# Chen001117/mappo

Hardware: AMD Instinct MI355X
Metric: agent-steps/sec (collect+GAE+PPO), MPE simple_spread 3-agent (higher is better)
Workload: dtype f32; 1 GPU; BASELINE configs[1]: MPE simple_spread shape, 3 agents, obs 18 / share_obs 54 / Discrete(5), n_rollout_threads=1024 in total (strong scaling: 1024 on rank 0 of 1), episode_length=25, MLP policy (mappo), ppo_epoch=10, num_mini_batch=1, lr 7e-4, env=synthetic; n_rollout_threads_global=1024, n_rollout_threads_rank0=1024, episode_length=25, num_agents=3, ppo_epoch=10, num_mini_batch=1, parallelism=dp1, rccl_ranks=0, exact_minibatch_order=False, hip_graph=True

## Files before the change

### include/mappo_hip.h

```cpp
#ifndef MAPPO_HIP_H
#define MAPPO_HIP_H

#include <stdint.h>

#ifdef __cplusplus
extern "C" {
#endif

typedef void *mappo_stream_t;

#define MAPPO_OK 0
#define MAPPO_EINVAL (-1)
#define MAPPO_ELAUNCH (-2)
#define MAPPO_ENOTIMPL (-3)

#define MAPPO_HIDDEN 64
#define MAPPO_MAX_IN_DIM 512
#define MAPPO_MAX_ACTIONS 32
#define MAPPO_MAX_LAYER_N 2

const char *mappo_last_error(void);
int mappo_abi_version(void);

typedef struct {
// ... 126 lines not shown
                       mappo_stream_t stream);
int mappo_critic_update(const float *params, const mappo_net_desc *desc , const float *share_obs,
                        const int32_t *rows, int64_t B, const float *v_old, const float *returns,
                        const float *active, const float *vn_state ,
                        const double *mb_moments , const mappo_ppo_cfg *cfg , float *slabs,
                        int64_t slab_stride, int64_t slab_col0, double *partials, float *wide_ws ,
                        int32_t n_blocks, mappo_stream_t stream);
int32_t mappo_dual_update_slabs(const mappo_net_desc *actor_desc , const mappo_net_desc *critic_desc , int64_t B);
int mappo_actor_critic_update(const float *actor_params, const mappo_net_desc *actor_desc , const float *obs,
                              const float *critic_params, const mappo_net_desc *critic_desc , const float *share_obs,
                              const int32_t *rows, int64_t B, const float *avail, const float *actions, const float *old_logp,
                              const float *adv, const float *active, const float *v_old, const float *returns,
                              const float *vn_state, const double *mb_moments, const mappo_ppo_cfg *cfg , float *slabs,
                              int64_t slab_stride, int64_t actor_col0, int64_t critic_col0, double *actor_partials,
                              double *critic_partials, mappo_stream_t stream);
int mappo_update_stats(const double *actor_partials, int32_t n_actor ,
                       const double *critic_partials, int32_t n_critic, const double *mb_moments,
                       const mappo_ppo_cfg *cfg , double *stats ,
                       double *acc ,
                       mappo_stream_t stream);

int mappo_mlp_features(const float *params, const mappo_net_desc *desc , const float *x, const int32_t *rows,
                       int64_t B, float *featT , mappo_stream_t stream);
int mappo_gru_forward(const float *params, const mappo_net_desc *desc , const float *featT, const float *h0,
                      const int32_t *h0_rows , const float *masks, const int32_t *rows ,
                      int32_t L, int32_t Nc, float *h_last ,
                      int32_t head_mode, float *out, const float *avail , int32_t deterministic,
                      uint64_t seed, uint64_t counter, const uint64_t *counter_dev, float *actions, float *logp,
                      mappo_stream_t stream);
int mappo_gru_step_dual(const float *actor_params, const mappo_net_desc *actor_desc , const float *actor_featT ,
// ... 94 lines not shown
```

### mappo_amd/_lib.py

```python
import ctypes as C
import os

import torch

_HERE = os.path.dirname(os.path.abspath(__file__))
LIB_PATH = os.environ.get("MAPPO_HIP_LIB") or os.path.join(_HERE, "libmappo_hip.so")

HIDDEN = 64
MAX_ACTIONS = 32
MAX_LAYER_N = 2


class NetDesc(C.Structure):
    _fields_ = [("in_dim", C.c_int32), ("hidden", C.c_int32), ("out_dim", C.c_int32), ("layer_N", C.c_int32),
                ("use_relu", C.c_int32), ("use_feature_norm", C.c_int32), ("recurrent", C.c_int32)]


class PpoCfg(C.Structure):
    _fields_ = [("clip_param", C.c_float), ("entropy_coef", C.c_float), ("value_loss_coef", C.c_float),
                ("huber_delta", C.c_float), ("use_huber_loss", C.c_int32), ("use_clipped_value_loss", C.c_int32),
                ("use_policy_active_masks", C.c_int32), ("use_value_active_masks", C.c_int32),
                ("use_valuenorm", C.c_int32), ("accumulate_partials", C.c_int32)]


# ... 32 lines not shown
                                        _I64, _I64, _P, _I64, _I64, _I64, _I32, _U64, _U64, _P, _P, _P, _P, _P, _P, _P, _P, _P, _I32, _P]),
    "mappo_mlp_backward_slabs": (_I32, [_I64]),
    "mappo_mlp_backward": (C.c_int, [_P, C.POINTER(NetDesc), _P, _P, _I64, _P, _P, _I64, _I64, _P, _P]),
    "mappo_wide_workspace_floats": (_I64, [_I64]),
    "mappo_wide_l1_slabs": (_I32, [_I64]),
    "mappo_wide_layout": (_I32, [C.POINTER(NetDesc), _I32]),
    "mappo_wide_l1_backward": (C.c_int, [_P, C.POINTER(NetDesc), _P, _P, _I64, _P, _P, _I64, _I64, _I32, _P]),
    "mappo_update_partials_bytes": (_I64, []),
    "mappo_actor_update": (C.c_int, [_P, C.POINTER(NetDesc), _P, _P, _I64, _P, _P, _P, _P, _P, _P, C.POINTER(PpoCfg), _P, _I64,
                                     _I64, _P, _P, _I32, _P]),
    "mappo_critic_update": (C.c_int, [_P, C.POINTER(NetDesc), _P, _P, _I64, _P, _P, _P, _P, _P, C.POINTER(PpoCfg), _P, _I64,
                                      _I64, _P, _P, _I32, _P]),
    "mappo_dual_update_slabs": (_I32, [C.POINTER(NetDesc), C.POINTER(NetDesc), _I64]),
    "mappo_actor_critic_update": (C.c_int, [_P, C.POINTER(NetDesc), _P, _P, C.POINTER(NetDesc), _P, _P, _I64, _P, _P, _P, _P, _P, _P, _P, _P, _P,
                                            C.POINTER(PpoCfg), _P, _I64, _I64, _I64, _P, _P, _P]),
    "mappo_update_stats": (C.c_int, [_P, _I32, _P, _I32, _P, C.POINTER(PpoCfg), _P, _P, _P]),
    "mappo_mlp_features": (C.c_int, [_P, C.POINTER(NetDesc), _P, _P, _I64, _P, _P]),
    "mappo_gru_forward": (C.c_int, [_P, C.POINTER(NetDesc), _P, _P, _P, _P, _P, _I32, _I32, _P, _I32, _P, _P, _I32, _U64, _U64,
                                    _P, _P, _P, _P]),
    "mappo_gru_step_dual": (C.c_int, [_P, C.POINTER(NetDesc), _P, _P, _P, _P, C.POINTER(NetDesc), _P, _P, _P, _P, _I32, _P, _I32, _U64, _U64,
                                      _P, _P, _P, _P, _P]),
    "mappo_recurrent_step_dual": (C.c_int, [_P, C.POINTER(NetDesc), _P, _P, _P, _P, C.POINTER(NetDesc), _P, _P, _P, _P, _I32, _P, _I32, _U64, _U64,
                                      _P, _P, _P, _P, _P]),
    "mappo_gru16_scratch_floats": (_I64, [_I32, _I32]),
    "mappo_gru16_blocked_floats": (_I64, [_I32, _I32]),
    "mappo_gru16_slabs": (_I32, [_I32, _I32]),
    "mappo_mlp_features_seq": (C.c_int, [_P, C.POINTER(NetDesc), _P, _P, _I32, _I32, _P, _P]),
    "mappo_gru16_forward_loss": (C.c_int, [_P, C.POINTER(NetDesc), _P, _I32, _P, _P, _P, _P, _I32, _I32, _I32] + [_P] * 9 +
                                 [C.POINTER(PpoCfg), _P, _P, _I64, _I64, _P, _P]),
    "mappo_gru16_backward": (C.c_int, [_P, C.POINTER(NetDesc), _P, _P, _I32, _I32, _P, _P, _P]),
# ... 45 lines not shown
```

### mappo_amd/algorithms/r_mappo/r_mappo.py

```python
import numpy as np
import os
import torch

from mappo_amd import ops
from mappo_amd.utils.util import to_device_f32
from mappo_amd.utils.valuenorm import ValueNorm


class R_MAPPO():
    def __init__(self, args, policy, device=torch.device("cuda"), dist_group=None):
        self.device = torch.device(device)
        self.tpdv = dict(dtype=torch.float32, device=self.device)
        self.policy = policy
        self.args = args

        self.clip_param = args.clip_param
        self.ppo_epoch = args.ppo_epoch
        self.num_mini_batch = args.num_mini_batch
        self.data_chunk_length = args.data_chunk_length
        self.value_loss_coef = args.value_loss_coef
        self.entropy_coef = args.entropy_coef
        self.max_grad_norm = args.max_grad_norm
        self.huber_delta = args.huber_delta

# ... 111 lines not shown
                na, nc = self._split_grid(n_slabs, pol.actor.desc.in_dim, pol.critic.desc.in_dim, B)
            if na:
                cur = torch.cuda.current_stream()
                if self._side_stream is None:
                    self._side_stream = torch.cuda.Stream(device=self.device)
                side = self._side_stream
                side.wait_stream(cur)
                with torch.cuda.stream(side):
                    ops.actor_update(pol.actor.flat, pol.actor.desc, src["obs"], rows, B, src["avail"], src["actions"],
                                     src["old_logp"], src["adv"], src["active"], self._mb_moments, cfg, slabs, P, 0, pa, na)
                ops.critic_update(pol.critic.flat, pol.critic.desc, src["share_obs"], rows, B, src["v_old"], src["returns"],
                                  src["active"], vn_state, self._mb_moments, cfg, slabs, P, pol.seg_bounds[1], pc, nc)
                cur.wait_stream(side)
                n_pa, n_pc = na, nc
            elif update_actor and self._dual_update and pol.can_dual_update():
                ops.actor_critic_update(pol.actor.flat, pol.actor.desc, src["obs"], pol.critic.flat, pol.critic.desc, src["share_obs"],
                                        rows, B, src["avail"], src["actions"], src["old_logp"], src["adv"], src["active"], src["v_old"],
                                        src["returns"], vn_state, self._mb_moments, cfg, slabs, P, 0, pol.seg_bounds[1], pa, pc)
                n_pa = n_pc = ops.dual_update_slabs(pol.actor.desc, pol.critic.desc, B)
                self._slab_rows = n_pa
            else:
                if update_actor:
                    ops.actor_update(pol.actor.flat, pol.actor.desc, src["obs"], rows, B, src["avail"], src["actions"],
                                     src["old_logp"], src["adv"], src["active"], self._mb_moments, cfg, slabs, P, 0, pa)
                ops.critic_update(pol.critic.flat, pol.critic.desc, src["share_obs"], rows, B, src["v_old"], src["returns"],
                                  src["active"], vn_state, self._mb_moments, cfg, slabs, P, pol.seg_bounds[1], pc)
                n_pa = n_pc = n_slabs
            if ep is None:
                ops.update_stats(pa if update_actor else None, n_pa, pc, n_pc, self._mb_moments, self._cfg, self._stats, self._acc)

        else:
            logits = self._buf("logits", (B, A))
            values = self._buf("values", (B,))
# ... 1 lines not shown
            ops.mlp_forward(pol.critic.flat, pol.critic.desc, src["share_obs"], rows, B, values)
            dlogits = self._buf("dlogits", (B, A))
            dvalues = self._buf("dvalues", (B,))
            ops.ppo_loss_fwd_bwd(logits, values, rows, src["avail"], src["actions"], src["old_logp"], src["adv"],
                                 src["active"], src["v_old"], src["returns"], vn_state, self._mb_moments, dlogits, dvalues,
                                 self._stats, self._cfg, self._bytes("loss_ws", lib.mappo_ppo_loss_workspace_bytes(B)))
            self._acc[:4].add_(self._stats[:4])
            if update_actor:
                ops.mlp_backward(pol.actor.flat, pol.actor.desc, src["obs"], rows, B, dlogits, slabs, P, 0)
            ops.mlp_backward(pol.critic.flat, pol.critic.desc, src["share_obs"], rows, B, dvalues, slabs, P, pol.seg_bounds[1])
        return slabs

    _actor_slabs_clean = True
    _actor_enabled = True
    _side_stream = None

    @staticmethod
    def _split_grid(n_slabs, d_actor, d_critic, B):
        if n_slabs < 256 or d_actor > 64 or d_critic > 64:
            return 0, 0
        tiles = (B + 31) // 32
        cost = lambda d: 1.0 + 0.25 * (d > 32)
        best = None
        for na in range(96, 161, 4):
            nc = 256 - na
            t = max(-(-tiles // (4 * na)) * cost(d_actor), -(-tiles // (4 * nc)) * cost(d_critic))
            if best is None or t < best[0]:
                best = (t, na, nc)
        return best[1], best[2]

# ... 59 lines not shown
        src, _ = self._buffer_sources(buffer, adv)
        self._zbuf.zero_()
        whole = self.num_mini_batch == 1 and not self._exact_order
        dp_graph = self._dist is not None and self._use_graph and whole and self._fused and self._dist.world_is_gpu
        key = (self._buffer_key(buffer), bool(update_actor))
        self._epochs = None
        if whole and self._fused and (self._dist is None or dp_graph) and not self._concurrent_update \
                and os.environ.get("MAPPO_EPOCH_BATCH", "1") != "0":
            self._epochs = dict(n=self.ppo_epoch, e=0, states=self._buf("vn_states", (self.ppo_epoch, 3)))
        if dp_graph:
            vn_state = self.value_normalizer.state if self._use_valuenorm else None
            self._moments(src, None, S, vn_state)
        for epoch in range(self.ppo_epoch):
            if self._epochs is not None:
                self._epochs["e"] = epoch
            if whole:
                batches = [(None, S)]
            else:
                batches = [(rows, rows.numel()) for rows in buffer.feed_forward_rows(self.num_mini_batch)]
            for rows, B in batches:
                if dp_graph:
                    gkey = key + (epoch,)
                    st = self._dp_graphs.get(gkey)
                    if st is None and self._dp_graphs.get(key) == "warm":
                        st = "warm"
                    if st == "warm":
                        torch.cuda.synchronize()
                        try:
                            g = torch.cuda.CUDAGraph()
                            with torch.cuda.graph(g, capture_error_mode="thread_local"):
# ... 1 lines not shown
                            self._dp_graphs[gkey] = st = g
                        except Exception as e:
                            import warnings
                            warnings.warn(f"hipGraph capture of the data-parallel update segment failed ({e}); launching eagerly")
                            torch.cuda.synchronize()
                            self._dp_graphs[gkey] = st = "off"
                    if st == "off":
                        st = None
                    if st is None:
                        self._update(src, rows, B, update_actor, moments_ready=True, part="kernels")
                    else:
                        st.replay()
                    self._update(src, rows, B, update_actor, moments_ready=True, part="optim")
                else:
                    self._update(src, rows, B, update_actor, moments_ready=whole and epoch > 0)
        if self._epochs is not None:
            n_rows = ops.dual_update_slabs(self.policy.actor.desc, self.policy.critic.desc, S) if (update_actor and self._dual_update and self.policy.can_dual_update()) \
                else ops.mlp_backward_slabs(S)
            ops.update_stats(self._pa if update_actor else None, n_rows, self._pc, n_rows, self._mb_moments, self._cfg, self._stats,
                             self._acc)
            self._epochs = None
        if dp_graph and self._dp_graphs.get(key) is None:
            self._dp_graphs[key] = "warm"
        if after_update:
            buffer.after_update()

    def compute_advantages(self, buffer):
        T = buffer.episode_length
        S = T * buffer.n_rollout_threads * buffer.num_agents
        adv = self._buf("adv", (S,))
# ... 61 lines not shown
```

### mappo_amd/csrc/mlp_impl.h

```cpp
#include "mlp_core.h"
#include <stdlib.h>

#ifdef MLP_TU_MAIN
extern "C" int64_t mappo_net_param_count(const mappo_net_desc *desc) {
  if (!desc) return -1;
  return net_offsets(*desc).total;
}
#endif

struct LdsMap {
  int w1, w2[MAPPO_MAX_LAYER_N], wh;
  int fn_w, fn_b, b1, ln1_w, ln1_b, b2[MAPPO_MAX_LAYER_N], ln2_w[MAPPO_MAX_LAYER_N], ln2_b[MAPPO_MAX_LAYER_N], bh;
  int scratch;
  int tiles, x_rows, wave_stride, total;
  int fn_size;
};


__host__ __device__ inline LdsMap lds_map(const mappo_net_desc &d, int n_waves) {
  LdsMap m;
  int p = 0;
  const bool xw = d.in_dim > MAXD;
  const int Dp = xw ? MAXD : ((d.in_dim + 1) & ~1);
  m.fn_size = xw ? ((d.in_dim + 63) / 64) * 64 : MAXD;
// ... 2314 lines not shown
  a.n_regions = (np > 1 && 2 * a.p_red + vec_floats <= tile_area) ? 2 : 1;
  MAPPO_REQUIRE(a.n_regions * a.p_red + vec_floats <= tile_area, "%s: reduction buffer too small", who);
  return MAPPO_OK;
}

extern "C" int32_t mappo_dual_update_slabs(const mappo_net_desc *actor_desc, const mappo_net_desc *critic_desc, int64_t B) {
  if (actor_desc && critic_desc && upd16_eligible(*actor_desc, true) && upd16_eligible(*critic_desc, false)) {
    int nA, nC;
    upd16_split(*actor_desc, *critic_desc, B, nA, nC);
    return nA > nC ? nA : nC;
  }
  int64_t n_tiles = (B + TS - 1) / TS;
  return (int32_t)(n_tiles < NUM_CU / 2 ? n_tiles : NUM_CU / 2);
}

extern "C" int mappo_actor_critic_update(const float *actor_params, const mappo_net_desc *actor_desc, const float *obs,
                                         const float *critic_params, const mappo_net_desc *critic_desc, const float *share_obs,
                                         const int32_t *rows, int64_t B, const float *avail, const float *actions,
                                         const float *old_logp, const float *adv, const float *active, const float *v_old,
                                         const float *returns, const float *vn_state, const double *mb_moments,
                                         const mappo_ppo_cfg *cfg, float *slabs, int64_t slab_stride, int64_t actor_col0,
                                         int64_t critic_col0, double *actor_partials, double *critic_partials,
                                         mappo_stream_t stream) {
  if (int rc = check_desc(actor_desc, "actor_critic_update")) return rc;
  if (int rc = check_desc(critic_desc, "actor_critic_update")) return rc;
  MAPPO_REQUIRE(actor_desc->in_dim <= MAXD && critic_desc->in_dim <= MAXD, "actor_critic_update: in_dim > %d takes the separate launches", MAXD);
  MAPPO_REQUIRE(actor_desc->layer_N == critic_desc->layer_N && actor_desc->use_relu == critic_desc->use_relu,
                "actor_critic_update: actor and critic must share layer_N and the activation");
  MAPPO_REQUIRE(critic_desc->out_dim == 1, "actor_critic_update: critic out_dim must be 1");
  MAPPO_REQUIRE(actor_params && critic_params && obs && share_obs && actions && old_logp && adv && active && v_old && returns && mb_moments &&
                    cfg && slabs && actor_partials && critic_partials && B > 0, "actor_critic_update: bad arguments");
  MAPPO_REQUIRE(!cfg->use_valuenorm || vn_state, "actor_critic_update: use_valuenorm needs vn_state");
  MAPPO_CLEAR_STICKY();
  if (upd16_eligible(*actor_desc, true) && upd16_eligible(*critic_desc, false)) {
    Dual16Args d = {};
    UpdArgs &a = d.a.u, &c = d.c.u;
    a.params = actor_params; a.x = obs; a.rows = rows; a.slabs = slabs; a.slab_stride = slab_stride; a.slab_col0 = actor_col0;
    a.desc = *actor_desc; a.B = B; a.avail = avail; a.actions = actions; a.old_logp = old_logp; a.adv = adv; a.active = active;
    a.mb_moments = mb_moments; a.partials = actor_partials; a.cfg = *cfg;
    c.params = critic_params; c.x = share_obs; c.rows = rows; c.slabs = slabs; c.slab_stride = slab_stride; c.slab_col0 = critic_col0;
    c.desc = *critic_desc; c.B = B; c.v_old = v_old; c.returns = returns; c.active = active; c.vn_state = vn_state;
    c.mb_moments = mb_moments; c.partials = critic_partials; c.cfg = *cfg;
    if (int rc = prep16(d.a, true, "actor_critic_update")) return rc;
    if (int rc = prep16(d.c, false, "actor_critic_update")) return rc;
    upd16_split(a.desc, c.desc, B, d.nA, d.nC);
#ifdef MLP_STAMPS
    a.stamps = c.stamps = g_stamp_host;
    a.stamps_waves = c.stamps_waves = g_stamp_waves_host;
#endif
    if (d.nA < d.nC) { d.c.zero_row0 = d.nA; d.c.zero_row1 = d.nC; d.c.zero_col0 = actor_col0; d.c.zero_cols = a.off.total; d.c.zero_partials = actor_partials; }
    if (d.nC < d.nA) { d.a.zero_row0 = d.nC; d.a.zero_row1 = d.nA; d.a.zero_col0 = critic_col0; d.a.zero_cols = c.off.total; d.a.zero_partials = critic_partials; }
    const size_t la = upd16_lds_floats(a.desc, true), lc = upd16_lds_floats(c.desc, false);
    const size_t lds_bytes = (la > lc ? la : lc) * sizeof(float);
    dim3 grid((unsigned)(d.nA + d.nC)), block(WAVE * UPD16_WAVES);
    const bool wa = a.desc.in_dim > 32, wc = c.desc.in_dim > 32, relu = a.desc.use_relu != 0;
    int rc;
    if (a.desc.layer_N == 0) rc = relu ? upd16d_inst<true, 0>(wa, wc, grid, block, lds_bytes, as_stream(stream), d) : upd16d_inst<false, 0>(wa, wc, grid, block, lds_bytes, as_stream(stream), d);
    else rc = relu ? upd16d_inst<true, 1>(wa, wc, grid, block, lds_bytes, as_stream(stream), d) : upd16d_inst<false, 1>(wa, wc, grid, block, lds_bytes, as_stream(stream), d);
    if (rc) return rc;
// ... 21 lines not shown
  a.stamps = c.stamps = nullptr;
#endif
  dim3 grid((unsigned)(d.nA + d.nC)), block(2 * WAVE * np);
  const bool wa = a.desc.in_dim > 32, wc = c.desc.in_dim > 32, relu = a.desc.use_relu != 0;
  int rc;
  switch (a.desc.layer_N) {
    case 0: rc = relu ? upd2d_inst<true, 0>(wa, wc, grid, block, lds_bytes, as_stream(stream), d) : upd2d_inst<false, 0>(wa, wc, grid, block, lds_bytes, as_stream(stream), d); break;
    case 1: rc = relu ? upd2d_inst<true, 1>(wa, wc, grid, block, lds_bytes, as_stream(stream), d) : upd2d_inst<false, 1>(wa, wc, grid, block, lds_bytes, as_stream(stream), d); break;
    default: rc = relu ? upd2d_inst<true, 2>(wa, wc, grid, block, lds_bytes, as_stream(stream), d) : upd2d_inst<false, 2>(wa, wc, grid, block, lds_bytes, as_stream(stream), d); break;
  }
  if (rc) return rc;
  MAPPO_CHECK_LAUNCH("actor_critic_update");
  return MAPPO_OK;
}

struct WideArgs {
  const float *params, *x;
  const int32_t *rows;
  const float *wide_ws;
  float *slabs;
  int64_t slab_stride, slab_col0;
  NetOff off;
  int64_t B;
  int D, use_feature_norm;
};

__global__ __launch_bounds__(256, 1) void wide_l1_bwd_kernel(WideArgs p) {
  extern __shared__ __align__(16) float lds[];
  const int lane = threadIdx.x & (WAVE - 1), wave = __builtin_amdgcn_readfirstlane((int)(threadIdx.x / WAVE)), l31 = lane & 31, half = lane >> 5;
  const int D = p.D, c0 = blockIdx.y * MAXD, kc = min(MAXD, D - c0);
// ... 220 lines not shown
```

### mappo_amd/csrc/mlp_upd16.h

```cpp
#pragma once
#include <utility>
#include <type_traits>

template <class F, int... I>
__device__ __forceinline__ void static_for_impl16(F &f, std::integer_sequence<int, I...>) { (f(std::integral_constant<int, I>{}), ...); }
template <int N, class F>
__device__ __forceinline__ void static_for16(F &&f) { static_for_impl16(f, std::make_integer_sequence<int, N>{}); }

#define UPD16_THREADS 512
#define RS16 68
#define HS16 80
#define DLS16 20

template <int LN, int HEAD, bool WIDE, bool XL1 = false>
struct L16 {
  static constexpr int CP = WIDE ? 16 : 8, NT = CP / 4, NBK = WIDE ? 4 : 2, XST = 16 * NBK + 4;
  static constexpr int W1 = 0;
  static constexpr int W2 = W1 + (XL1 ? 0 : HID * 4 * CP);
  static constexpr int W2T = W2 + (LN > 0 ? HID * HID : 0);
  static constexpr int WH = W2T + (LN > 0 ? HID * HID : 0);
  __host__ __device__ static constexpr int w1_at(int f, int r) { return ((f >> 4) * NT + ((r % CP) >> 2)) * 256 + ((r / CP) * 16 + (f & 15)) * 4 + (r & 3); }
  static constexpr int B1 = WH + (HEAD == 1 ? 16 * HS16 : HID), B2 = B1 + HID, BH = B2 + HID;
  static constexpr int FN_W = BH + 16, FN_B = FN_W + HID, G1 = FN_B + HID, T1 = G1 + HID, G2 = T1 + HID, T2 = G2 + HID;
  static constexpr int TILES = T2 + HID;
// ... 6 lines not shown
  static constexpr int EPI4 = 1024 + N_WAVES * 4 * 256 + PMAX, EPI8 = 1024 + N_WAVES * 8 * 256 + PMAX;
  static constexpr int TILE_AREA0 = N_WAVES * WAVE_STRIDE > EPI4 ? N_WAVES * WAVE_STRIDE : EPI4;
  static constexpr int TILE_AREA = TILE_AREA0 < EPI8 && TILES + EPI8 <= LDS_CAP && 2 * (TILES + TILE_AREA0) > LDS_CAP ? EPI8 : TILE_AREA0;
  static constexpr int TOTAL = TILES + TILE_AREA;
  static constexpr int CH = (EPI8 <= TILE_AREA) ? 8 : 4;
  static_assert(1024 + N_WAVES * CH * 256 + PMAX <= TILE_AREA, "epilogue buffers do not fit the tile area");
  static_assert(TILES % 4 == 0, "the epilogue's chunk buffer and flat gradient are read and written 16 bytes at a time");
};

struct Upd16Args {
  UpdArgs u;
  int zero_row0, zero_row1;
  int64_t zero_col0;
  int zero_cols;
  double *zero_partials;
};

__device__ __forceinline__ float xhalf_max(float v) {
  const unsigned u = __float_as_uint(v);
  const auto r = __builtin_amdgcn_permlane32_swap(u, u, false, false);
  return fmaxf(__uint_as_float(r[0]), __uint_as_float(r[1]));
}
__device__ __forceinline__ float xrow_max(float v) {
  const unsigned u = __float_as_uint(v);
  const auto r = __builtin_amdgcn_permlane16_swap(u, u, false, false);
  return fmaxf(__uint_as_float(r[0]), __uint_as_float(r[1]));
}
__device__ __forceinline__ float quad_max16(float v) { return xhalf_max(xrow_max(v)); }

__device__ __forceinline__ f32x4 ld4(const float *p) {
  const float4 t = *reinterpret_cast<const float4 *>(p);
  f32x4 r; r[0] = t.x; r[1] = t.y; r[2] = t.z; r[3] = t.w;
  return r;
}
__device__ __forceinline__ void st4(float *p, const f32x4 &v) { *reinterpret_cast<float4 *>(p) = make_float4(v[0], v[1], v[2], v[3]); }

template <bool RELU>
__device__ __forceinline__ void act_ln_fwd16(f32x4 (&a)[4], float &mean, float &rstd, uint32_t &pos) {
  f32x4 s = {0.f, 0.f, 0.f, 0.f};
#pragma unroll
  for (int b = 0; b < 4; ++b) {
#pragma unroll
    for (int i = 0; i < 4; ++i) a[b][i] = act_fwd<RELU>(a[b][i]);
    s += a[b];
  }
  mean = quad_sum16((s[0] + s[1]) + (s[2] + s[3])) * (1.f / HID);
  const f32x4 mean4 = {mean, mean, mean, mean};
  f32x4 v = {0.f, 0.f, 0.f, 0.f};
#pragma unroll
  for (int b = 0; b < 4; ++b) { a[b] -= mean4; v += a[b] * a[b]; }
  pos = 0u;
  rstd = __builtin_amdgcn_rsqf(quad_sum16((v[0] + v[1]) + (v[2] + v[3])) * (1.f / HID) + LN_EPS);
  const f32x4 rstd4 = {rstd, rstd, rstd, rstd};
#pragma unroll
  for (int b = 0; b < 4; ++b) a[b] *= rstd4;
}

template <bool RELU>
__device__ __forceinline__ void ln_act_bwd16(f32x4 (&d)[4], const f32x4 (&xh)[4], float mean, float rstd, uint32_t pos) {
  (void)pos;
  f32x4 s1 = {0.f, 0.f, 0.f, 0.f}, s2 = {0.f, 0.f, 0.f, 0.f};
#pragma unroll
  for (int b = 0; b < 4; ++b) { s1 += d[b]; s2 += d[b] * xh[b]; }
  const float m1 = quad_sum16((s1[0] + s1[1]) + (s1[2] + s1[3])) * (1.f / HID);
  const float m2 = quad_sum16((s2[0] + s2[1]) + (s2[2] + s2[3])) * (1.f / HID);
  const float inv_rstd = __builtin_amdgcn_rcpf(rstd);
  const float c0 = -m1 * rstd, c1 = -m2 * rstd;
  const f32x4 c04 = {c0, c0, c0, c0}, c14 = {c1, c1, c1, c1}, rstd4 = {rstd, rstd, rstd, rstd};
// ... 54 lines not shown
    }
  }
}

__device__ __forceinline__ float col_sum16(const float *U, int stride, int col) {
  float s0 = 0.f, s1 = 0.f;
#pragma unroll
  for (int s = 0; s < 16; s += 2) { s0 += U[s * stride + col]; s1 += U[(s + 1) * stride + col]; }
  return s0 + s1;
}

template <bool WIDE>
struct Prefetch16 {
  float xv[WIDE ? 16 : 8];
  float f0, f1, f2, f3;
  uint32_t dead;
  int n_valid;
  bool flat;
};

template <int HEAD, bool WIDE>
__device__ __forceinline__ void prefetch16(Prefetch16<WIDE> &pf, const UpdArgs &p, int64_t tile, int64_t n_tiles, int D, int C, int A,
                                           int lane, int n, int q) {
  constexpr int NV = WIDE ? 16 : 8;
  int64_t base = tile * 16;
  int nv = (tile < n_tiles) ? (int)min((int64_t)16, p.B - base) : 0;
  if (HEAD == 3 && p.seq_nc > 0 && tile < n_tiles) {
    const int n_ct = (p.seq_nc + 15) >> 4;
    const int64_t t = tile / n_ct;
    const int j0 = (int)(tile - t * n_ct) * 16;
    base = t * p.seq_nc + j0;
    nv = min(16, p.seq_nc - j0);
  }
  pf.n_valid = nv;
  pf.flat = p.rows == nullptr && nv == 16 && (((uintptr_t)(p.x + base * D)) & 15) == 0;
  pf.f0 = pf.f1 = pf.f2 = pf.f3 = 0.f;
  pf.dead = 0u;
  if (nv == 0) return;
  if (pf.flat) {
    const __amdgpu_buffer_rsrc_t rx = __builtin_amdgcn_make_buffer_rsrc((void *)(p.x + base * D), 0, 16 * D * 4, 0x00020000);
#pragma unroll
    for (int j = 0; j < NV / 4; ++j) {
      const f32x4 t = __builtin_amdgcn_raw_buffer_load_b128(rx, lane * 16, 1024 * j, 0);
      pf.xv[4 * j + 0] = t[0]; pf.xv[4 * j + 1] = t[1]; pf.xv[4 * j + 2] = t[2]; pf.xv[4 * j + 3] = t[3];
    }
    if constexpr (HEAD == 1) {
      pf.f0 = (p.actions + base)[n]; pf.f1 = (p.old_logp + base)[n]; pf.f2 = (p.adv + base)[n]; pf.f3 = (p.active + base)[n];
      if (p.avail) {
        const __amdgpu_buffer_rsrc_t ra = __builtin_amdgcn_make_buffer_rsrc((void *)(p.avail + base * A), 0, 16 * A * 4, 0x00020000);
        float v[4];
#pragma unroll
        for (int i = 0; i < 4; ++i) v[i] = __builtin_amdgcn_raw_buffer_load_b32(ra, (n * A + q) * 4, 16 * i, 0);
#pragma unroll
        for (int i = 0; i < 4; ++i) pf.dead |= ((4 * i + q < A && v[i] == 0.f) ? 1u : 0u) << i;
      }
    } else if constexpr (HEAD == 2) {
      pf.f0 = (p.v_old + base)[n]; pf.f1 = (p.returns + base)[n]; pf.f2 = (p.active + base)[n];
    }
    return;
  }
  const bool ok = n < nv;
  const int64_t row = ok ? (p.rows ? (int64_t)p.rows[base + n] : base + n) : 0;
  int qo = q;
  asm volatile("" : "+v"(qo));
  const float *src = p.x + row * D;
#pragma unroll
  for (int t = 0; t < NV; ++t) pf.xv[t] = src[min(qo * C + t, D - 1)];
  if constexpr (HEAD == 1) {
    pf.f0 = p.actions[row]; pf.f1 = p.old_logp[row]; pf.f2 = p.adv[row]; pf.f3 = p.active[row];
    if (p.avail) {
      const float *av = p.avail + row * A;
      float v[4];
#pragma unroll
      for (int i = 0; i < 4; ++i) v[i] = av[min(4 * i + qo, A - 1)];
#pragma unroll
      for (int i = 0; i < 4; ++i) pf.dead |= ((4 * i + q < A && v[i] == 0.f) ? 1u : 0u) << i;
    }
  } else if constexpr (HEAD == 2) {
    pf.f0 = p.v_old[row]; pf.f1 = p.returns[row]; pf.f2 = p.active[row];
  }
}

template <int HEAD>
__device__ __forceinline__ void prefetch16x(Prefetch16<true> &pf, const UpdArgs &p, const float *z1, int64_t tile, int64_t n_tiles, int A,
                                            int n, int q) {
  const int64_t base = tile * 16;
  const int nv = (tile < n_tiles) ? (int)min((int64_t)16, p.B - base) : 0;
  pf.n_valid = nv;
  pf.flat = true;
  pf.f0 = pf.f1 = pf.f2 = pf.f3 = 0.f;
  pf.dead = 0u;
// ... 128 lines not shown
  static_assert(!XL1 || WIDE, "XL1 uses the 16-register prefetch block");
  constexpr int NV = WIDE ? 16 : 8, NBK = WIDE ? 4 : 2;
  const UpdArgs &p = P.u;
  typedef L16<LN, HEAD, WIDE, XL1> M;
  const float *z1 = XL1 ? p.wide_ws + 66 * ((p.B + 15) & ~(int64_t)15) : nullptr;
  const NetOff &o = p.off;
  const int lane = threadIdx.x & (WAVE - 1), n = lane & 15, q = lane >> 4;
  const int wave = __builtin_amdgcn_readfirstlane((int)(threadIdx.x / WAVE)), n_waves = blockDim.x / WAVE;
  const int D = p.desc.in_dim, A = p.desc.out_dim, C = (D + 3) >> 2;
  const bool fnorm = p.desc.use_feature_norm != 0;
  const float inv_D = 1.0f / (float)D;
  const bool seq = HEAD == 3 && p.seq_nc > 0;
  const int64_t n_tiles = seq ? (p.B / p.seq_nc) * ((p.seq_nc + 15) >> 4) : (p.B + 15) / 16;
  const int64_t tile_stride = (int64_t)nb * n_waves;
  const int64_t tile0 = (int64_t)wave * nb + bid;
  Prefetch16<WIDE> pf;
  if constexpr (XL1) prefetch16x<HEAD>(pf, p, z1, tile0, n_tiles, A, n, q);
  else prefetch16<HEAD, WIDE>(pf, p, tile0, n_tiles, D, C, A, lane, n, q);
  STAMP_DECL

  {
    static_assert(UPD16_THREADS == 512, "staging assumes 64 rows x 8 threads");
    const float *__restrict__ g = p.params;
    const int tid = threadIdx.x, f8 = tid >> 3, part = tid & 7;
    const int vid = tid >> 6, ve = tid & 63;
    float w1r[M::CP / 2], w2r[8], whr[8], vecv, b1raw, b2raw = 0.f, bhraw = 0.f;
    if constexpr (!XL1) {
#pragma unroll
      for (int j = 0; j < M::CP / 2; ++j) {
        const int r = part + 8 * j, k = (r / M::CP) * C + (r % M::CP);
        w1r[j] = g[o.w1 + f8 * D + min(k, D - 1)];
      }
    }
// ... 128 lines not shown
      const float *db = p.dHT + min(tile0, n_tiles - 1) * 1024 + lane * 4;
#pragma unroll
      for (int b = 0; b < 4; ++b) dh_next[b] = ld4(db + b * 256);
    } else {
      const float *dcol = p.dHT + min(tile0 * 16 + n, p.B - 1);
#pragma unroll
      for (int b = 0; b < 4; ++b)
#pragma unroll
        for (int i = 0; i < 4; ++i) dh_next[b][i] = dcol[(int64_t)(16 * b + 4 * q + i) * p.B];
    }
  }
  for (int64_t tile = tile0; tile < n_tiles; tile += tile_stride) {
    const int n_valid = pf.n_valid;
    const bool live = n < n_valid;
    const float c0 = pf.f0, c1 = pf.f1, c2 = pf.f2, c3 = pf.f3;
    const uint32_t cdead = pf.dead;
    f32x4 xh[4];
    float mean1, rstd1, mean2 = 0.f, rstd2 = 1.f;
    uint32_t pos1, pos2 = 0u;
    if constexpr (XL1) {
#pragma unroll
      for (int b = 0; b < 4; ++b) { xh[b][0] = pf.xv[4 * b]; xh[b][1] = pf.xv[4 * b + 1]; xh[b][2] = pf.xv[4 * b + 2]; xh[b][3] = pf.xv[4 * b + 3]; }
      STAMP(1);
    } else {
    float x0[NV];
    {
      if (pf.flat) {
#pragma unroll
        for (int j = 0; j < NV / 4; ++j)
          *reinterpret_cast<float4 *>(Ux + 4 * (lane + 64 * j)) = make_float4(pf.xv[4 * j], pf.xv[4 * j + 1], pf.xv[4 * j + 2], pf.xv[4 * j + 3]);
        wave_lds_sync();
#pragma unroll
        for (int t = 0; t < NV; ++t) x0[t] = rawp[t];
        wave_lds_sync();
      } else {
#pragma unroll
        for (int t = 0; t < NV; ++t) x0[t] = pf.xv[t];
      }
      float s4[4] = {0.f, 0.f, 0.f, 0.f};
#pragma unroll
      for (int t = 0; t < NV; ++t) { x0[t] = (t < nvl) ? x0[t] : 0.f; s4[t & 3] += x0[t]; }
      if (fnorm) {
        const float mean = quad_sum16((s4[0] + s4[1]) + (s4[2] + s4[3])) * inv_D;
        float v4[4] = {0.f, 0.f, 0.f, 0.f};
#pragma unroll
        for (int t = 0; t < NV; ++t) { x0[t] -= mean; v4[t & 3] += x0[t] * x0[t]; }
        const float var = quad_sum16(((v4[0] + v4[1]) + (v4[2] + v4[3])) - n_empty * mean * mean);
        const float rstd = __builtin_amdgcn_rsqf(fmaxf(var, 0.f) * inv_D + LN_EPS);
#pragma unroll
        for (int t = 0; t < NV; ++t) x0[t] *= rstd;
      }
#pragma unroll
      for (int j = 0; j < NV / 4; ++j)
        *reinterpret_cast<float4 *>(x0p + 4 * j) = make_float4(x0[4 * j], x0[4 * j + 1], x0[4 * j + 2], x0[4 * j + 3]);
    }

    STAMP(1);
#pragma unroll
    for (int bo = 0; bo < 4; ++bo) xh[bo] = ld4(lds + M::B1 + 16 * bo + 4 * q);
#pragma unroll
    for (int tc = 0; tc < NV / 4; ++tc) {
      const int nk = C - 4 * tc;
      if (nk > 0) {
        f32x4 a[4];
#pragma unroll
        for (int bo = 0; bo < 4; ++bo) a[bo] = ld4(lds + M::W1 + ((bo * M::NT + tc) * 64 + lane) * 4);
// ... 1 lines not shown
          constexpr int K = decltype(kc)::value;
#pragma unroll
          for (int i = 0; i < K; ++i)
#pragma unroll
            for (int bo = 0; bo < 4; ++bo) xh[bo] = mfma16(a[bo][i], x0[4 * tc + i], xh[bo]);
        };
        if (nk >= 4) ksteps(std::integral_constant<int, 4>{});
        else if (nk == 3) ksteps(std::integral_constant<int, 3>{});
        else if (nk == 2) ksteps(std::integral_constant<int, 2>{});
        else ksteps(std::integral_constant<int, 1>{});
      }
    }
    }
    STAMP(2);
    if constexpr (XL1) prefetch16x<HEAD>(pf, p, z1, tile + tile_stride, n_tiles, A, n, q);
    else prefetch16<HEAD, WIDE>(pf, p, tile + tile_stride, n_tiles, D, C, A, lane, n, q);
    f32x4 dh[HEAD == 3 ? 4 : 1];
    if constexpr (HEAD == 3) {
      if constexpr (DH_AHEAD) {
#pragma unroll
        for (int b = 0; b < 4; ++b) dh[b] = dh_next[b];
        if (seq) {
          const float *db = p.dHT + min(tile + tile_stride, n_tiles - 1) * 1024 + lane * 4;
#pragma unroll
          for (int b = 0; b < 4; ++b) dh_next[b] = ld4(db + b * 256);
        } else {
          const float *dcol = p.dHT + min((tile + tile_stride) * 16 + n, p.B - 1);
#pragma unroll
          for (int b = 0; b < 4; ++b)
#pragma unroll
            for (int i = 0; i < 4; ++i) dh_next[b][i] = dcol[(int64_t)(16 * b + 4 * q + i) * p.B];
// ... 325 lines not shown
```

### mappo_amd/ops.py

```python
import ctypes as C

import torch

from . import _lib
from ._lib import NetDesc, PpoCfg


def _ptr(t, dtype=torch.float32, allow_none=False):
    if t is None:
        if allow_none:
            return None
        raise ValueError("tensor required")
    if not t.is_cuda:
        raise _lib.MappoHipError("mappo_amd ops need tensors in HBM (cuda/hip device); got a CPU tensor — "
                                 "there is no CPU fallback")
    if t.dtype != dtype:
        raise TypeError(f"expected {dtype}, got {t.dtype}")
    if not t.is_contiguous():
        raise ValueError("tensor must be contiguous")
    return C.c_void_p(t.data_ptr())


def _stream():
    return C.c_void_p(torch.cuda.current_stream().cuda_stream)
# ... 303 lines not shown
    rc = _lib.load().mappo_critic_update(_ptr(params), C.byref(desc), _ptr(share_obs), _ptr(rows, torch.int32, allow_none=True),
                                         int(B), _ptr(v_old), _ptr(returns), _ptr(active), _ptr(vn_state, allow_none=True),
                                         _ptr(mb_moments, torch.float64), C.byref(cfg), _ptr(slabs), int(slab_stride),
                                         int(slab_col0), _ptr(partials, torch.float64), _ptr(ws, allow_none=True), int(n_blocks),
                                         _stream())
    _lib.check(rc, "mappo_critic_update")
    _wide(desc, share_obs, rows, B, slabs, slab_stride, slab_col0, params, ws, PRODUCER_CRITIC_UPDATE)


def dual_update_slabs(actor_desc, critic_desc, B):
    return int(_lib.load().mappo_dual_update_slabs(C.byref(actor_desc), C.byref(critic_desc), int(B)))


def actor_critic_update(actor_params, actor_desc, obs, critic_params, critic_desc, share_obs, rows, B, avail, actions, old_logp, adv,
                        active, v_old, returns, vn_state, mb_moments, cfg, slabs, slab_stride, actor_col0, critic_col0,
                        actor_partials, critic_partials):
    rc = _lib.load().mappo_actor_critic_update(_ptr(actor_params), C.byref(actor_desc), _ptr(obs), _ptr(critic_params), C.byref(critic_desc),
                                               _ptr(share_obs), _ptr(rows, torch.int32, allow_none=True), int(B),
                                               _ptr(avail, allow_none=True), _ptr(actions), _ptr(old_logp), _ptr(adv), _ptr(active),
                                               _ptr(v_old), _ptr(returns), _ptr(vn_state, allow_none=True),
                                               _ptr(mb_moments, torch.float64), C.byref(cfg), _ptr(slabs), int(slab_stride),
                                               int(actor_col0), int(critic_col0), _ptr(actor_partials, torch.float64),
                                               _ptr(critic_partials, torch.float64), _stream())
    _lib.check(rc, "mappo_actor_critic_update")


def update_stats(actor_partials, n_actor, critic_partials, n_critic, mb_moments, cfg, stats, acc=None):
    rc = _lib.load().mappo_update_stats(_ptr(actor_partials, torch.float64, allow_none=True), int(n_actor),
                                        _ptr(critic_partials, torch.float64), int(n_critic), _ptr(mb_moments, torch.float64),
                                        C.byref(cfg), _ptr(stats, torch.float64), _ptr(acc, torch.float64, allow_none=True), _stream())
    _lib.check(rc, "mappo_update_stats")


def mlp_features(params, desc, x, rows, B, featT):
    rc = _lib.load().mappo_mlp_features(_ptr(params), C.byref(desc), _ptr(x), _ptr(rows, torch.int32, allow_none=True), int(B),
                                        _ptr(featT), _stream())
    _lib.check(rc, "mappo_mlp_features")


# ... 177 lines not shown
```

Before: 76.69 million agent-steps/s.

## Cache feature-normalized inputs across PPO epochs in fused actor-critic update

In whole-batch PPO updates, the first epoch writes the feature-normalized layer-0 input (per tile, lane-packed) into a cache buffer, and later epochs read it with buffer loads. This skips reloading raw obs and recomputing the input LayerNorm in each of the remaining epochs. The avail-action dead mask is now computed lazily from prefetched raw bits. A pair4 helper also changes how mean and rstd are broadcast. In exchange the epoch-0 pass does extra stores and needs cache memory, and the path only applies when feature norm is on and rows is null.

```diff
diff --git a/include/mappo_hip.h b/include/mappo_hip.h
--- a/include/mappo_hip.h
+++ b/include/mappo_hip.h
@@ -164,6 +164,15 @@
                               const float *vn_state, const double *mb_moments, const mappo_ppo_cfg *cfg , float *slabs,
                               int64_t slab_stride, int64_t actor_col0, int64_t critic_col0, double *actor_partials,
                               double *critic_partials, mappo_stream_t stream);
+int64_t mappo_update_x0_cache_floats(const mappo_net_desc *desc , int64_t B);
+int mappo_actor_critic_update_x0(const float *actor_params, const mappo_net_desc *actor_desc , const float *obs,
+                                 const float *critic_params, const mappo_net_desc *critic_desc , const float *share_obs,
+                                 const int32_t *rows, int64_t B, const float *avail, const float *actions, const float *old_logp,
+                                 const float *adv, const float *active, const float *v_old, const float *returns,
+                                 const float *vn_state, const double *mb_moments, const mappo_ppo_cfg *cfg , float *slabs,
+                                 int64_t slab_stride, int64_t actor_col0, int64_t critic_col0, double *actor_partials,
+                                 double *critic_partials, float *actor_x0, float *critic_x0, int32_t x0_mode,
+                                 mappo_stream_t stream);
 int mappo_update_stats(const double *actor_partials, int32_t n_actor ,
                        const double *critic_partials, int32_t n_critic, const double *mb_moments,
                        const mappo_ppo_cfg *cfg , double *stats ,
diff --git a/mappo_amd/_lib.py b/mappo_amd/_lib.py
--- a/mappo_amd/_lib.py
+++ b/mappo_amd/_lib.py
@@ -70,6 +70,9 @@
     "mappo_dual_update_slabs": (_I32, [C.POINTER(NetDesc), C.POINTER(NetDesc), _I64]),
     "mappo_actor_critic_update": (C.c_int, [_P, C.POINTER(NetDesc), _P, _P, C.POINTER(NetDesc), _P, _P, _I64, _P, _P, _P, _P, _P, _P, _P, _P, _P,
                                             C.POINTER(PpoCfg), _P, _I64, _I64, _I64, _P, _P, _P]),
+    "mappo_update_x0_cache_floats": (_I64, [C.POINTER(NetDesc), _I64]),
+    "mappo_actor_critic_update_x0": (C.c_int, [_P, C.POINTER(NetDesc), _P, _P, C.POINTER(NetDesc), _P, _P, _I64, _P, _P, _P, _P, _P, _P, _P, _P,
+                                               _P, C.POINTER(PpoCfg), _P, _I64, _I64, _I64, _P, _P, _P, _P, _I32, _P]),
     "mappo_update_stats": (C.c_int, [_P, _I32, _P, _I32, _P, C.POINTER(PpoCfg), _P, _P, _P]),
     "mappo_mlp_features": (C.c_int, [_P, C.POINTER(NetDesc), _P, _P, _I64, _P, _P]),
     "mappo_gru_forward": (C.c_int, [_P, C.POINTER(NetDesc), _P, _P, _P, _P, _P, _I32, _I32, _P, _I32, _P, _P, _I32, _U64, _U64,
diff --git a/mappo_amd/algorithms/r_mappo/r_mappo.py b/mappo_amd/algorithms/r_mappo/r_mappo.py
--- a/mappo_amd/algorithms/r_mappo/r_mappo.py
+++ b/mappo_amd/algorithms/r_mappo/r_mappo.py
@@ -149,9 +149,15 @@
                 cur.wait_stream(side)
                 n_pa, n_pc = na, nc
             elif update_actor and self._dual_update and pol.can_dual_update():
+                x0_mode, x0c = 0, None
+                if rows is None and self._x0_epoch is not None:
+                    x0_mode = 1 if self._x0_epoch == 0 else 2
+                    x0c = (self._buf("x0_actor", (ops.update_x0_cache_floats(pol.actor.desc, B),)),
+                           self._buf("x0_critic", (ops.update_x0_cache_floats(pol.critic.desc, B),)))
                 ops.actor_critic_update(pol.actor.flat, pol.actor.desc, src["obs"], pol.critic.flat, pol.critic.desc, src["share_obs"],
                                         rows, B, src["avail"], src["actions"], src["old_logp"], src["adv"], src["active"], src["v_old"],
-                                        src["returns"], vn_state, self._mb_moments, cfg, slabs, P, 0, pol.seg_bounds[1], pa, pc)
+                                        src["returns"], vn_state, self._mb_moments, cfg, slabs, P, 0, pol.seg_bounds[1], pa, pc,
+                                        x0_caches=x0c, x0_mode=x0_mode)
                 n_pa = n_pc = ops.dual_update_slabs(pol.actor.desc, pol.critic.desc, B)
                 self._slab_rows = n_pa
             else:
@@ -183,6 +189,7 @@
     _actor_slabs_clean = True
     _actor_enabled = True
     _side_stream = None
+    _x0_epoch = None
 
     @staticmethod
     def _split_grid(n_slabs, d_actor, d_critic, B):
@@ -272,6 +279,7 @@
         for epoch in range(self.ppo_epoch):
             if self._epochs is not None:
                 self._epochs["e"] = epoch
+            self._x0_epoch = epoch if whole else None
             if whole:
                 batches = [(None, S)]
             else:
@@ -303,6 +311,7 @@
                     self._update(src, rows, B, update_actor, moments_ready=True, part="optim")
                 else:
                     self._update(src, rows, B, update_actor, moments_ready=whole and epoch > 0)
+        self._x0_epoch = None
         if self._epochs is not None:
             n_rows = ops.dual_update_slabs(self.policy.actor.desc, self.policy.critic.desc, S) if (update_actor and self._dual_update and self.policy.can_dual_update()) \
                 else ops.mlp_backward_slabs(S)
diff --git a/mappo_amd/csrc/mlp_impl.h b/mappo_amd/csrc/mlp_impl.h
--- a/mappo_amd/csrc/mlp_impl.h
+++ b/mappo_amd/csrc/mlp_impl.h
@@ -2352,14 +2352,16 @@
   return (int32_t)(n_tiles < NUM_CU / 2 ? n_tiles : NUM_CU / 2);
 }
 
-extern "C" int mappo_actor_critic_update(const float *actor_params, const mappo_net_desc *actor_desc, const float *obs,
-                                         const float *critic_params, const mappo_net_desc *critic_desc, const float *share_obs,
-                                         const int32_t *rows, int64_t B, const float *avail, const float *actions,
-                                         const float *old_logp, const float *adv, const float *active, const float *v_old,
-                                         const float *returns, const float *vn_state, const double *mb_moments,
-                                         const mappo_ppo_cfg *cfg, float *slabs, int64_t slab_stride, int64_t actor_col0,
-                                         int64_t critic_col0, double *actor_partials, double *critic_partials,
-                                         mappo_stream_t stream) {
+static int64_t x0_cache_floats(const mappo_net_desc &d, int64_t B) { return (B + 15) / 16 * 64 * (d.in_dim > 32 ? 16 : 8); }
+
+static int actor_critic_update_impl(const float *actor_params, const mappo_net_desc *actor_desc, const float *obs,
+                                    const float *critic_params, const mappo_net_desc *critic_desc, const float *share_obs,
+                                    const int32_t *rows, int64_t B, const float *avail, const float *actions,
+                                    const float *old_logp, const float *adv, const float *active, const float *v_old,
+                                    const float *returns, const float *vn_state, const double *mb_moments,
+                                    const mappo_ppo_cfg *cfg, float *slabs, int64_t slab_stride, int64_t actor_col0,
+                                    int64_t critic_col0, double *actor_partials, double *critic_partials,
+                                    float *actor_x0, float *critic_x0, int32_t x0_mode, mappo_stream_t stream) {
   if (int rc = check_desc(actor_desc, "actor_critic_update")) return rc;
   if (int rc = check_desc(critic_desc, "actor_critic_update")) return rc;
   MAPPO_REQUIRE(actor_desc->in_dim <= MAXD && critic_desc->in_dim <= MAXD, "actor_critic_update: in_dim > %d takes the separate launches", MAXD);
@@ -2381,6 +2383,10 @@
     c.mb_moments = mb_moments; c.partials = critic_partials; c.cfg = *cfg;
     if (int rc = prep16(d.a, true, "actor_critic_update")) return rc;
     if (int rc = prep16(d.c, false, "actor_critic_update")) return rc;
+    if (x0_mode != 0 && rows == nullptr) {
+      if (a.desc.use_feature_norm && actor_x0) { d.a.x0c = actor_x0; d.a.x0c_mode = x0_mode; }
+      if (c.desc.use_feature_norm && critic_x0) { d.c.x0c = critic_x0; d.c.x0c_mode = x0_mode; }
+    }
     upd16_split(a.desc, c.desc, B, d.nA, d.nC);
 #ifdef MLP_STAMPS
     a.stamps = c.stamps = g_stamp_host;
@@ -2432,6 +2438,43 @@
   return MAPPO_OK;
 }
 
+extern "C" int mappo_actor_critic_update(const float *actor_params, const mappo_net_desc *actor_desc, const float *obs,
+                                         const float *critic_params, const mappo_net_desc *critic_desc, const float *share_obs,
+                                         const int32_t *rows, int64_t B, const float *avail, const float *actions,
+                                         const float *old_logp, const float *adv, const float *active, const float *v_old,
+                                         const float *returns, const float *vn_state, const double *mb_moments,
+                                         const mappo_ppo_cfg *cfg, float *slabs, int64_t slab_stride, int64_t actor_col0,
+                                         int64_t critic_col0, double *actor_partials, double *critic_partials,
+                                         mappo_stream_t stream) {
+  return actor_critic_update_impl(actor_params, actor_desc, obs, critic_params, critic_desc, share_obs, rows, B, avail, actions, old_logp,
+                                  adv, active, v_old, returns, vn_state, mb_moments, cfg, slabs, slab_stride, actor_col0, critic_col0,
+                                  actor_partials, critic_partials, nullptr, nullptr, 0, stream);
+}
+
+extern "C" int64_t mappo_update_x0_cache_floats(const mappo_net_desc *desc, int64_t B) {
+  if (!desc || B < 0) {
+    mappo_set_error("update_x0_cache_floats: bad arguments");
+    return MAPPO_EINVAL;
+  }
+  return x0_cache_floats(*desc, B);
+}
+
+extern "C" int mappo_actor_critic_update_x0(const float *actor_params, const mappo_net_desc *actor_desc, const float *obs,
+                                            const float *critic_params, const mappo_net_desc *critic_desc, const float *share_obs,
+                                            const int32_t *rows, int64_t B, const float *avail, const float *actions,
+                                            const float *old_logp, const float *adv, const float *active, const float *v_old,
+                                            const float *returns, const float *vn_state, const double *mb_moments,
+                                            const mappo_ppo_cfg *cfg, float *slabs, int64_t slab_stride, int64_t actor_col0,
+                                            int64_t critic_col0, double *actor_partials, double *critic_partials,
+                                            float *actor_x0, float *critic_x0, int32_t x0_mode, mappo_stream_t stream) {
+  MAPPO_REQUIRE(x0_mode >= 0 && x0_mode <= 2, "actor_critic_update_x0: x0_mode %d", x0_mode);
+  MAPPO_REQUIRE(x0_mode == 0 || (actor_x0 && critic_x0 && (((uintptr_t)actor_x0 | (uintptr_t)critic_x0) & 15) == 0),
+                "actor_critic_update_x0: x0 caches must be non-null and 16-byte aligned");
+  return actor_critic_update_impl(actor_params, actor_desc, obs, critic_params, critic_desc, share_obs, rows, B, avail, actions, old_logp,
+                                  adv, active, v_old, returns, vn_state, mb_moments, cfg, slabs, slab_stride, actor_col0, critic_col0,
+                                  actor_partials, critic_partials, actor_x0, critic_x0, x0_mode, stream);
+}
+
 struct WideArgs {
   const float *params, *x;
   const int32_t *rows;
diff --git a/mappo_amd/csrc/mlp_upd16.h b/mappo_amd/csrc/mlp_upd16.h
--- a/mappo_amd/csrc/mlp_upd16.h
+++ b/mappo_amd/csrc/mlp_upd16.h
@@ -44,6 +44,8 @@
   int64_t zero_col0;
   int zero_cols;
   double *zero_partials;
+  float *x0c;
+  int x0c_mode;
 };
 
 __device__ __forceinline__ float xhalf_max(float v) {
@@ -65,6 +67,12 @@
 }
 __device__ __forceinline__ void st4(float *p, const f32x4 &v) { *reinterpret_cast<float4 *>(p) = make_float4(v[0], v[1], v[2], v[3]); }
 
+__device__ __forceinline__ f32x4 pair4(float v) {
+  float w = v;
+  asm volatile("" : "+v"(w));
+  return f32x4{v, w, v, w};
+}
+
 template <bool RELU>
 __device__ __forceinline__ void act_ln_fwd16(f32x4 (&a)[4], float &mean, float &rstd, uint32_t &pos) {
   f32x4 s = {0.f, 0.f, 0.f, 0.f};
@@ -75,13 +83,13 @@
     s += a[b];
   }
   mean = quad_sum16((s[0] + s[1]) + (s[2] + s[3])) * (1.f / HID);
-  const f32x4 mean4 = {mean, mean, mean, mean};
+  const f32x4 mean4 = pair4(mean);
   f32x4 v = {0.f, 0.f, 0.f, 0.f};
 #pragma unroll
   for (int b = 0; b < 4; ++b) { a[b] -= mean4; v += a[b] * a[b]; }
   pos = 0u;
   rstd = __builtin_amdgcn_rsqf(quad_sum16((v[0] + v[1]) + (v[2] + v[3])) * (1.f / HID) + LN_EPS);
-  const f32x4 rstd4 = {rstd, rstd, rstd, rstd};
+  const f32x4 rstd4 = pair4(rstd);
 #pragma unroll
   for (int b = 0; b < 4; ++b) a[b] *= rstd4;
 }
@@ -166,14 +174,24 @@
 struct Prefetch16 {
   float xv[WIDE ? 16 : 8];
   float f0, f1, f2, f3;
+  uint32_t av[4];
   uint32_t dead;
   int n_valid;
   bool flat;
 };
 
+template <bool WIDE>
+__device__ __forceinline__ uint32_t prefetch_dead16(const Prefetch16<WIDE> &pf, int A, int q) {
+  const uint32_t m = pf.flat ? ~0u : 0x7fffffffu;
+  uint32_t dead = 0u;
+#pragma unroll
+  for (int i = 0; i < 4; ++i) dead |= ((4 * i + q < A && (pf.av[i] & m) == 0u) ? 1u : 0u) << i;
+  return dead;
+}
+
 template <int HEAD, bool WIDE>
-__device__ __forceinline__ void prefetch16(Prefetch16<WIDE> &pf, const UpdArgs &p, int64_t tile, int64_t n_tiles, int D, int C, int A,
-                                           int lane, int n, int q) {
+__device__ __forceinline__ void prefetch16(Prefetch16<WIDE> &pf, const UpdArgs &p, const float *x0c, int64_t tile, int64_t n_tiles, int D,
+                                           int C, int A, int lane, int n, int q) {
   constexpr int NV = WIDE ? 16 : 8;
   int64_t base = tile * 16;
   int nv = (tile < n_tiles) ? (int)min((int64_t)16, p.B - base) : 0;
@@ -189,44 +207,38 @@
   pf.f0 = pf.f1 = pf.f2 = pf.f3 = 0.f;
   pf.dead = 0u;
   if (nv == 0) return;
-  if (pf.flat) {
+  int qo = q;
+  asm volatile("" : "+v"(qo));
+  int64_t row;
+  if (x0c) {
+    const __amdgpu_buffer_rsrc_t rc = __builtin_amdgcn_make_buffer_rsrc((void *)(x0c + tile * 64 * NV), 0, 64 * NV * 4, 0x00020000);
+#pragma unroll
+    for (int j = 0; j < NV / 4; ++j) {
+      const f32x4 t = __builtin_amdgcn_raw_buffer_load_b128(rc, lane * NV * 4, 16 * j, 0);
+      pf.xv[4 * j + 0] = t[0]; pf.xv[4 * j + 1] = t[1]; pf.xv[4 * j + 2] = t[2]; pf.xv[4 * j + 3] = t[3];
+    }
+    row = min(base + n, p.B - 1);
+  } else if (pf.flat) {
     const __amdgpu_buffer_rsrc_t rx = __builtin_amdgcn_make_buffer_rsrc((void *)(p.x + base * D), 0, 16 * D * 4, 0x00020000);
 #pragma unroll
     for (int j = 0; j < NV / 4; ++j) {
       const f32x4 t = __builtin_amdgcn_raw_buffer_load_b128(rx, lane * 16, 1024 * j, 0);
       pf.xv[4 * j + 0] = t[0]; pf.xv[4 * j + 1] = t[1]; pf.xv[4 * j + 2] = t[2]; pf.xv[4 * j + 3] = t[3];
     }
-    if constexpr (HEAD == 1) {
-      pf.f0 = (p.actions + base)[n]; pf.f1 = (p.old_logp + base)[n]; pf.f2 = (p.adv + base)[n]; pf.f3 = (p.active + base)[n];
-      if (p.avail) {
-        const __amdgpu_buffer_rsrc_t ra = __builtin_amdgcn_make_buffer_rsrc((void *)(p.avail + base * A), 0, 16 * A * 4, 0x00020000);
-        float v[4];
-#pragma unroll
-        for (int i = 0; i < 4; ++i) v[i] = __builtin_amdgcn_raw_buffer_load_b32(ra, (n * A + q) * 4, 16 * i, 0);
-#pragma unroll
-        for (int i = 0; i < 4; ++i) pf.dead |= ((4 * i + q < A && v[i] == 0.f) ? 1u : 0u) << i;
-      }
-    } else if constexpr (HEAD == 2) {
-      pf.f0 = (p.v_old + base)[n]; pf.f1 = (p.returns + base)[n]; pf.f2 = (p.active + base)[n];
-    }
-    return;
-  }
-  const bool ok = n < nv;
-  const int64_t row = ok ? (p.rows ? (int64_t)p.rows[base + n] : base + n) : 0;
-  int qo = q;
-  asm volatile("" : "+v"(qo));
-  const float *src = p.x + row * D;
-#pragma unroll
-  for (int t = 0; t < NV; ++t) pf.xv[t] = src[min(qo * C + t, D - 1)];
+    row = base + n;
+  } else {
+    const bool ok = n < nv;
+    row = ok ? (p.rows ? (int64_t)p.rows[base + n] : base + n) : 0;
+    const float *src = p.x + row * D;
+#pragma unroll
+    for (int t = 0; t < NV; ++t) pf.xv[t] = src[min(qo * C + t, D - 1)];
+  }
   if constexpr (HEAD == 1) {
     pf.f0 = p.actions[row]; pf.f1 = p.old_logp[row]; pf.f2 = p.adv[row]; pf.f3 = p.active[row];
     if (p.avail) {
       const float *av = p.avail + row * A;
-      float v[4];
-#pragma unroll
-      for (int i = 0; i < 4; ++i) v[i] = av[min(4 * i + qo, A - 1)];
-#pragma unroll
-      for (int i = 0; i < 4; ++i) pf.dead |= ((4 * i + q < A && v[i] == 0.f) ? 1u : 0u) << i;
+#pragma unroll
+      for (int i = 0; i < 4; ++i) pf.av[i] = __float_as_uint(av[min(4 * i + qo, A - 1)]);
     }
   } else if constexpr (HEAD == 2) {
     pf.f0 = p.v_old[row]; pf.f1 = p.returns[row]; pf.f2 = p.active[row];
@@ -385,9 +397,11 @@
   const int64_t n_tiles = seq ? (p.B / p.seq_nc) * ((p.seq_nc + 15) >> 4) : (p.B + 15) / 16;
   const int64_t tile_stride = (int64_t)nb * n_waves;
   const int64_t tile0 = (int64_t)wave * nb + bid;
+  const int x0m = (XL1 || HEAD == 3 || !P.x0c) ? 0 : P.x0c_mode;
+  const float *x0rd = x0m == 2 ? P.x0c : nullptr;
   Prefetch16<WIDE> pf;
   if constexpr (XL1) prefetch16x<HEAD>(pf, p, z1, tile0, n_tiles, A, n, q);
-  else prefetch16<HEAD, WIDE>(pf, p, tile0, n_tiles, D, C, A, lane, n, q);
+  else prefetch16<HEAD, WIDE>(pf, p, x0rd, tile0, n_tiles, D, C, A, lane, n, q);
   STAMP_DECL
 
   {
@@ -546,7 +560,7 @@
     const int n_valid = pf.n_valid;
     const bool live = n < n_valid;
     const float c0 = pf.f0, c1 = pf.f1, c2 = pf.f2, c3 = pf.f3;
-    const uint32_t cdead = pf.dead;
+    const uint32_t cdead = XL1 ? pf.dead : (p.avail ? prefetch_dead16(pf, A, q) : 0u);
     f32x4 xh[4];
     float mean1, rstd1, mean2 = 0.f, rstd2 = 1.f;
     uint32_t pos1, pos2 = 0u;
@@ -556,7 +570,10 @@
       STAMP(1);
     } else {
     float x0[NV];
-    {
+    if (x0m == 2) {
+#pragma unroll
+      for (int t = 0; t < NV; ++t) x0[t] = pf.xv[t];
+    } else {
       if (pf.flat) {
 #pragma unroll
         for (int j = 0; j < NV / 4; ++j)
@@ -582,6 +599,13 @@
 #pragma unroll
         for (int t = 0; t < NV; ++t) x0[t] *= rstd;
       }
+      if (x0m == 1) {
+        float *dst = P.x0c + (tile * 64 + lane) * NV;
+#pragma unroll
+        for (int j = 0; j < NV / 4; ++j) *reinterpret_cast<float4 *>(dst + 4 * j) = make_float4(x0[4 * j], x0[4 * j + 1], x0[4 * j + 2], x0[4 * j + 3]);
+      }
+    }
+    {
 #pragma unroll
       for (int j = 0; j < NV / 4; ++j)
         *reinterpret_cast<float4 *>(x0p + 4 * j) = make_float4(x0[4 * j], x0[4 * j + 1], x0[4 * j + 2], x0[4 * j + 3]);
@@ -613,7 +637,7 @@
     }
     STAMP(2);
     if constexpr (XL1) prefetch16x<HEAD>(pf, p, z1, tile + tile_stride, n_tiles, A, n, q);
-    else prefetch16<HEAD, WIDE>(pf, p, tile + tile_stride, n_tiles, D, C, A, lane, n, q);
+    else prefetch16<HEAD, WIDE>(pf, p, x0rd, tile + tile_stride, n_tiles, D, C, A, lane, n, q);
     f32x4 dh[HEAD == 3 ? 4 : 1];
     if constexpr (HEAD == 3) {
       if constexpr (DH_AHEAD) {
diff --git a/mappo_amd/ops.py b/mappo_amd/ops.py
--- a/mappo_amd/ops.py
+++ b/mappo_amd/ops.py
@@ -341,15 +341,26 @@
 
 def actor_critic_update(actor_params, actor_desc, obs, critic_params, critic_desc, share_obs, rows, B, avail, actions, old_logp, adv,
                         active, v_old, returns, vn_state, mb_moments, cfg, slabs, slab_stride, actor_col0, critic_col0,
-                        actor_partials, critic_partials):
-    rc = _lib.load().mappo_actor_critic_update(_ptr(actor_params), C.byref(actor_desc), _ptr(obs), _ptr(critic_params), C.byref(critic_desc),
-                                               _ptr(share_obs), _ptr(rows, torch.int32, allow_none=True), int(B),
-                                               _ptr(avail, allow_none=True), _ptr(actions), _ptr(old_logp), _ptr(adv), _ptr(active),
-                                               _ptr(v_old), _ptr(returns), _ptr(vn_state, allow_none=True),
-                                               _ptr(mb_moments, torch.float64), C.byref(cfg), _ptr(slabs), int(slab_stride),
-                                               int(actor_col0), int(critic_col0), _ptr(actor_partials, torch.float64),
-                                               _ptr(critic_partials, torch.float64), _stream())
+                        actor_partials, critic_partials, x0_caches=None, x0_mode=0):
+    lib = _lib.load()
+    args = (_ptr(actor_params), C.byref(actor_desc), _ptr(obs), _ptr(critic_params), C.byref(critic_desc),
+            _ptr(share_obs), _ptr(rows, torch.int32, allow_none=True), int(B),
+            _ptr(avail, allow_none=True), _ptr(actions), _ptr(old_logp), _ptr(adv), _ptr(active),
+            _ptr(v_old), _ptr(returns), _ptr(vn_state, allow_none=True),
+            _ptr(mb_moments, torch.float64), C.byref(cfg), _ptr(slabs), int(slab_stride),
+            int(actor_col0), int(critic_col0), _ptr(actor_partials, torch.float64), _ptr(critic_partials, torch.float64))
+    if x0_mode:
+        xa, xc = x0_caches
+        assert xa.numel() >= update_x0_cache_floats(actor_desc, B) and xc.numel() >= update_x0_cache_floats(critic_desc, B)
+        rc = lib.mappo_actor_critic_update_x0(*args, _ptr(xa), _ptr(xc), int(x0_mode), _stream())
+        _lib.check(rc, "mappo_actor_critic_update_x0")
+        return
+    rc = lib.mappo_actor_critic_update(*args, _stream())
     _lib.check(rc, "mappo_actor_critic_update")
+
+
+def update_x0_cache_floats(desc, B):
+    return int(_lib.load().mappo_update_x0_cache_floats(C.byref(desc), int(B)))
 
 
 def update_stats(actor_partials, n_actor, critic_partials, n_critic, mb_moments, cfg, stats, acc=None):
```

Result: no change. 77.34 million agent-steps/s (median of 6 runs) (+0.9%).
